# Viasat/nhd

Hardware: AMD Instinct MI355X
Metric: pod-placement filter-and-score throughput (pod x node fit-and-score evaluations/s; placement decisions/s under commit semantics in mode_b) (higher is better)
Workload: dtype u64 bitmaps + int32 table look-ups (f64 NIC arithmetic in the request digest)

## Files before the change

__graft_entry__.py:

```python
import os
import subprocess
import sys

ROOT = os.path.dirname(os.path.abspath(__file__))
if ROOT not in sys.path:
    sys.path.insert(0, ROOT)


def build() -> None:
    from nhd_amd import build as b
    b.build_lib()
    oracle_mk = os.path.join(ROOT, "oracle", "Makefile")
    if os.path.exists(oracle_mk):
        subprocess.check_call(["make", "-s", "-C", os.path.join(ROOT, "oracle")])
    from tests import harness
    harness.lib()
    from tests.harness import explain_twin
    explain_twin.lib()
    from tests.harness import headroom_twin
    headroom_twin.lib()
    headroom_twin.wave_lib()
    from tests.harness import headroom_limit_twin
    headroom_limit_twin.lib()
    from tests.harness import headroom_general_twin
    headroom_general_twin.lib()
    headroom_general_twin.wave_lib()
    from tests.harness import candidates_twin
    candidates_twin.lib()
    candidates_twin.pick_lib()
    from tests.harness import candidates_general_twin
    candidates_general_twin.lib()
    candidates_general_twin.wave_lib()
    import nhd_amd
    from nhd_amd import _lib
    lib = _lib.load()
    assert lib.nhdfit_abi_version() == _lib.ABI_VERSION


def smoke() -> None:
    import numpy as np
    from nhd_amd import matcher
    from workload import refmodel, synth
    from oracle import nhd_oracle as O

    spec = synth.make_cluster(3, n_nodes=192)
    nl = spec.build_nodes()
    pods, groups = synth.make_pods(3, n_pods=24)
    tops = [refmodel.make_topology(s) for s in pods]
    m = matcher.HipMatcher(device=0, clock=lambda: spec.clock_now)
    got = m.FindNodes(nl, tops)
    placed = 0
    for top, res in zip(tops, got):
        want = O.find_node(nl, top, spec.clock_now)
        if want[0] is None:
            assert res == (None,), (res, want)
        else:
            placed += 1
            assert res[0] == want[0] and res[1]["gpu"] == tuple(want[1]["gpu"]) and \
                res[1]["cpu"] == tuple(want[1]["cpu"]) and res[1]["nic"] == [tuple(x) for x in want[1]["nic"]], (res, want)
    assert placed > 0
    from nhd_amd.engine import winner_index
    reqs = m.packer.digest_many(tops)
    score, _, _ = m.engine.find(reqs, spec.clock_now, want_bitmap=True, want_map=True)
    names = list(nl)
    for s, res in zip(score.tolist(), got):
        assert (names[winner_index(s) - m.engine.global_base] if s else None) == res[0], (s, res)
    st = m.engine.stats()
    print(f"smoke ok: {len(tops)} pods x {len(nl)} nodes, {placed} placed; single-launch finds {st.small_finds}, step kernel {st.fit_ms_last * 1e3:.1f} us")


if __name__ == "__main__":
    build()
    if "--smoke" in sys.argv:
        smoke()
```

nhd_amd/csrc/fit_core.h:

```cpp
#pragma once
#include <stdint.h>
#include "../../include/nhdfit.h"

#if defined(__HIPCC__)
#define NHD_HD __host__ __device__ __forceinline__
#else
#define NHD_HD inline
#endif

namespace nhdfit {

constexpr int kMaxG      = NHDFIT_MAX_GROUPS;
constexpr int kTile      = NHDFIT_TILE;
constexpr int kMaxHpRows = 1024;
constexpr int kWClasses  = 4;
constexpr double kMinBusySecs = 30.0;
constexpr uint32_t kMinXCap = 32;

NHD_HD uint32_t align16(uint32_t x) { return (x + 15u) & ~15u; }
NHD_HD uint32_t wc_stride_of(uint32_t W) { return 2 * W * 8 + 16; }
NHD_HD uint32_t x_stride_of(uint32_t W) { return W == 2 ? 16u : W * 8 + 16; }

struct Layout {
    uint32_t W;
// ... 80 lines not shown
template <> struct req_traits<nhdfit_req> {
    static constexpr int kG = NHDFIT_MAX_GROUPS;
    static constexpr bool kBig = false;
    using Key = int16_t;
    static constexpr int kMaxTuples = 1024;
    using Mapping = nhdfit_mapping;
    using WidePlacement = nhdfit_wide_placement;
};
template <> struct req_traits<nhdfit_big_req> {
    static constexpr int kG = NHDFIT_BIG_MAX_GROUPS;
    static constexpr bool kBig = true;
    using Key = int32_t;
    static constexpr int kMaxTuples = NHDFIT_BIG_MAX_TUPLES;
    using Mapping = nhdfit_big_mapping;
    using WidePlacement = nhdfit_big_placement;
};
static_assert(sizeof(nhdfit_big_req) == 256 && sizeof(nhdfit_big_mapping) == 36 && sizeof(nhdfit_big_placement) == 904, "record sizes of include/nhdfit.h");
NHD_HD bool req_valid(const nhdfit_big_req& r) {
    return (r.map_type == NHDFIT_MAP_NUMA || r.map_type == NHDFIT_MAP_PCI) && r.n_groups >= 1 &&
           r.n_groups <= (uint32_t)NHDFIT_BIG_MAX_GROUPS;
}

NHD_HD void pod_sums(const nhdfit_req& r, PodSums& s) {
    s.G = r.n_groups;
    s.W = 1u << s.G;
    s.full = s.W - 1;
    s.misc_smt = r.misc_smt;
    s.misc_nosmt = r.misc_nosmt;
    for (uint32_t S = 0; S < s.W; ++S) {
        uint32_t g = 0, a = 0, b = 0;
        for (uint32_t i = 0; i < s.G; ++i)
            if (S >> i & 1) { g += r.gpus[i]; a += r.cpu_smt[i]; b += r.cpu_nosmt[i]; }
        s.gpu[S] = g; s.cpu_smt[S] = a; s.cpu_nosmt[S] = b;
    }
}

NHD_HD PodHeader pod_header(const nhdfit_req& r) {
    PodHeader h;
    h.hp_req = r.hugepages_gb;
    h.groups = r.groups;
    h.flags = 0;
    if (req_valid(r)) {
        h.flags |= kPodValid;
        uint32_t g = 0;
        for (uint32_t i = 0; i < r.n_groups; ++i) g += r.gpus[i];
        if (g) h.flags |= kPodNeedGpu;
        if (r.map_type == NHDFIT_MAP_PCI) h.flags |= kPodPci;
        if (r.flags & NHDFIT_RF_INITIAL_FILTER) h.flags |= kPodFilter;
        h.flags |= r.n_groups << kPodGroupsShift;
    }
    return h;
}

NHD_HD uint32_t entry_w(const PodSums& s, uint32_t u, bool smt, uint32_t c, uint32_t m) {
    const uint32_t* sum = smt ? s.cpu_smt : s.cpu_nosmt;
    const uint32_t extra = m ? (smt ? s.misc_smt : s.misc_nosmt) : 0;
    uint32_t out = 0;
    for (uint32_t p = 0; p < s.W; ++p)
        if (sum[u ? p : (~p & s.full)] + extra <= c) out |= 1u << p;
    return out;
}

NHD_HD uint32_t entry_a(const PodSums& s, uint32_t u, uint32_t f) {
    uint32_t a = 0;
    for (uint32_t p = 0; p < s.W; ++p)
        if (s.gpu[u ? p : (~p & s.full)] <= f) a |= 1u << p;
    return a;
}

static_assert(kMaxG == 4, "the disj() masks below enumerate subsets of four groups");
template <uint32_t TERMS>
NHD_HD uint32_t dunion_n(uint32_t a, uint32_t b) {
    uint32_t out = 0;
#if defined(__HIP_DEVICE_COMPILE__)
#pragma unroll
#endif
    for (uint32_t S = 0; S < TERMS; ++S) {
        const uint32_t disj = ((S & 1) ? 0x5555u : 0xFFFFu) & ((S & 2) ? 0x3333u : 0xFFFFu) &
                              ((S & 4) ? 0x0F0Fu : 0xFFFFu) & ((S & 8) ? 0x00FFu : 0xFFFFu);
        if (b >> S & 1) out |= (a & disj) << S;
    }
    return out;
}
NHD_HD uint32_t dunion(uint32_t a, uint32_t b, uint32_t W) {
    (void)W;
    return dunion_n<1u << kMaxG>(a, b);
}

NHD_HD bool block_fits(const nhdfit_req& r, double cap, uint32_t S) {
    double rx = cap, tx = cap;
    for (uint32_t i = 0; i < r.n_groups; ++i)
        if (S >> i & 1) { rx = rx - r.rx[i]; tx = tx - r.tx[i]; }
    return !(rx < 0) && !(tx < 0);
}

template <uint32_t WW>
NHD_HD void class_cover_w(const nhdfit_req& r, double cap, uint32_t W, uint32_t G, uint16_t cover[kMaxG + 1]) {
    uint32_t fit = 1;
    for (uint32_t S = 1; S < W; ++S)
        if (block_fits(r, cap, S)) fit |= 1u << S;
    cover[0] = 1;
    for (uint32_t n = 1; n <= (uint32_t)kMaxG; ++n)
        cover[n] = (n <= G) ? (uint16_t)dunion_n<WW>(cover[n - 1], fit) : cover[G];
}
NHD_HD void class_cover(const nhdfit_req& r, double cap, uint32_t W, uint32_t G, uint16_t cover[kMaxG + 1]) {
    class_cover_w<1u << kMaxG>(r, cap, W, G, cover);
}

NHD_HD uint32_t size_le_mask(uint32_t W, uint32_t limit) {
    const uint32_t by_size = limit == 0 ? 0x0001u : limit == 1 ? 0x0117u : limit == 2 ? 0x177Fu : limit == 3 ? 0x7FFFu : 0xFFFFu;
    return by_size & ((1u << W) - 1u);
}

struct SigDict {
    const uint32_t* sig_off;
    const uint32_t* pool_off;
    const uint8_t*  pool_glimit;
    const nhdfit_cc* cc;
    uint32_t nsig;
};

template <uint32_t WW>
NHD_HD uint32_t sig_reach_w(const SigDict& d, uint32_t sig, const uint16_t* cover, uint32_t W) {
    uint32_t reach = 1;
    for (uint32_t pl = d.sig_off[sig]; pl < d.sig_off[sig + 1]; ++pl) {
        uint32_t pool = 1;
        for (uint32_t k = d.pool_off[pl]; k < d.pool_off[pl + 1]; ++k) {
            uint32_t n = d.cc[k].cnt > kMaxG ? kMaxG : d.cc[k].cnt;
            pool = dunion_n<WW>(pool, cover[d.cc[k].cls * (kMaxG + 1) + n]);
        }
        if (d.pool_glimit[pl] != NHDFIT_GLIMIT_NONE) pool &= size_le_mask(W, d.pool_glimit[pl]);
        reach = dunion_n<WW>(reach, pool);
    }
    return reach;
}
NHD_HD uint32_t sig_reach(const SigDict& d, uint32_t sig, const uint16_t* cover, uint32_t W) {
    return sig_reach_w<1u << kMaxG>(d, sig, cover, W);
}

NHD_HD uint32_t entry_r(uint32_t reach, uint32_t W, uint32_t u) {
    if (u) return reach & 0xFFFFu;
    uint32_t r = reach & 0xFFFFu;
    r = (r & 0x5555u) << 1 | (r >> 1 & 0x5555u);
    r = (r & 0x3333u) << 2 | (r >> 2 & 0x3333u);
    r = (r & 0x0F0Fu) << 4 | (r >> 4 & 0x0F0Fu);
    r = (r & 0x00FFu) << 8 | (r >> 8 & 0x00FFu);
    return r >> (16 - W);
}

NHD_HD bool hp_bit(const PodHeader& h, uint32_t k) {
    if (!(h.flags & kPodValid)) return false;
    return h.hp_req <= (int32_t)k - 1;
}
NHD_HD bool gx_bit(const PodHeader& h, uint32_t g, const uint64_t* group_sets) {
    if (g == 0) return false;
    const uint32_t gs = (g - 1) >> 1, active = (g - 1) & 1;
    if (!(h.flags & kPodFilter)) return true;
    return active && (group_sets[gs] & h.groups) != 0;
}

struct NodeIdx {
    uint32_t w0, w1;
    uint32_t f0, f1;
    uint32_t hp;
    uint32_t gx;
    uint32_t nogpu;
};

NHD_HD NodeIdx node_index(const nhdfit_plane0& a, const nhdfit_plane1& b, const nhdfit_plane2& c, const nhdfit_plane4& e,
                          uint32_t fc_dim, uint32_t fg_dim, uint32_t ngs) {
    NodeIdx n;
    const uint32_t smt = (c.flags & NHDFIT_NF_SMT) ? fc_dim : 0;
    uint32_t c0 = popc64(a.t0[0] & b.t1[0]), c1 = popc64(a.t0[1] & b.t1[1]);
    c0 = c0 < fc_dim ? c0 : fc_dim - 1;
    c1 = c1 < fc_dim ? c1 : fc_dim - 1;
    n.w0 = smt + c0;
    n.w1 = smt + c1;
    uint32_t f0 = popc32(c.gpu_free & ~c.gpu_numa1), f1 = popc32(c.gpu_free & c.gpu_numa1);
    n.f0 = f0 < fg_dim ? f0 : fg_dim - 1;
    n.f1 = f1 < fg_dim ? f1 : fg_dim - 1;
    int32_t hp = c.hp_free;
    hp = hp < -1 ? -1 : hp;
    hp = hp > kMaxHpRows - 2 ? kMaxHpRows - 2 : hp;
    n.hp = (uint32_t)(hp + 1);
    const uint32_t gs = e.group_set < ngs ? e.group_set : 0;
    n.gx = (c.flags & NHDFIT_NF_MAINTENANCE) ? 0u : 1u + 2u * gs + ((c.flags & NHDFIT_NF_ACTIVE) ? 1u : 0u);
    n.nogpu = (c.flags & NHDFIT_NF_HAS_GPU) ? 0u : 1u;
    return n;
}

NHD_HD uint64_t xkey(uint32_t u, uint32_t f, uint32_t sig_numa, uint32_t sig_pci) {
    return (1ull << 63) | ((uint64_t)u << 62) | ((uint64_t)f << 32) | ((uint64_t)sig_numa << 16) | (uint64_t)sig_pci;
}
NHD_HD uint32_t xkey_u(uint64_t k) { return (uint32_t)(k >> 62) & 1u; }
NHD_HD uint32_t xkey_f(uint64_t k) { return (uint32_t)(k >> 32) & 0xFFu; }
NHD_HD uint32_t xkey_sig_numa(uint64_t k) { return (uint32_t)(k >> 16) & 0xFFFFu; }
NHD_HD uint32_t xkey_sig_pci(uint64_t k) { return (uint32_t)k & 0xFFFFu; }

struct alignas(16) NodeRec {
    uint16_t w0, w1, x0, x1;
    uint16_t gx;
    uint16_t hp;
    uint16_t flags;
    uint16_t cc;
};
static_assert(sizeof(NodeRec) == 16, "one 16-byte load per node");
static_assert(kMaxHpRows <= 1024, "NodeRec::hp keeps ten bits for the row index");
constexpr uint16_t kRecNoGpu = 1;
NHD_HD uint32_t rec_hp(const NodeRec& r) { return r.hp & 1023u; }
NHD_HD uint32_t rec_pos(const NodeRec& r) { return r.hp >> 10; }

NHD_HD uint32_t pair_c_row(uint32_t cc, uint32_t D);
NHD_HD NodeRec make_record(const NodeIdx& n, uint32_t x0, uint32_t x1, const Layout& L, uint32_t pos, uint32_t crow_D = 0) {
    NodeRec r;
    r.w0 = (uint16_t)((L.hot_wc0 + n.w0 * L.wc_stride) >> 3);
    r.w1 = (uint16_t)((L.hot_wc1 + n.w1 * L.wc_stride) >> 3);
    r.x0 = (uint16_t)((L.hot_x + x0 * L.x_stride) >> 3);
    r.x1 = (uint16_t)((L.hot_x + x1 * L.x_stride) >> 3);
    r.gx = (uint16_t)((L.hot_gx + n.gx * 8) >> 3);
    r.hp = (uint16_t)(n.hp | (pos & 63u) << 10);
    r.flags = (uint16_t)(n.nogpu ? kRecNoGpu : 0);
    const uint32_t smt = n.w0 >= L.fc_dim ? 1u : 0u;
    r.cc = (uint16_t)((n.w0 - smt * L.fc_dim) | (n.w1 - smt * L.fc_dim) << 7 | smt << 14);
    if (crow_D) r.flags = (uint16_t)(r.flags | pair_c_row(r.cc, crow_D) << 1);
    return r;
}
NHD_HD NodeRec dead_record(const Layout& L, uint32_t pos) {
    NodeRec r;
    r.w0 = (uint16_t)(L.hot_wc0 >> 3); r.w1 = (uint16_t)(L.hot_wc1 >> 3);
    r.x0 = r.x1 = (uint16_t)(L.hot_x >> 3);
    r.gx = (uint16_t)(L.hot_gx >> 3);
    r.hp = (uint16_t)((pos & 63u) << 10); r.flags = 0; r.cc = 0;
    return r;
}

NHD_HD uint32_t req_max_demand(const nhdfit_req& r) {
    uint32_t a = r.misc_smt, b = r.misc_nosmt;
    for (uint32_t i = 0; i < r.n_groups && i < (uint32_t)kMaxG; ++i) { a += r.cpu_smt[i]; b += r.cpu_nosmt[i]; }
    return a > b ? a : b;
}
NHD_HD uint32_t pair_dim(uint32_t max_demand, uint32_t fc_dim) { return max_demand + 1 < fc_dim ? max_demand + 1 : fc_dim; }
NHD_HD uint32_t pair_c_row(uint32_t cc, uint32_t D) {
    const uint32_t c0 = cc & 127u, c1 = (cc >> 7) & 127u, smt = cc >> 14;
    return ((smt * D + (c0 < D ? c0 : D - 1)) * D + (c1 < D ? c1 : D - 1));
}

inline double busy_threshold(double now) {
    constexpr uint64_t kSign = 1ull << 63, kMaxBits = 0x7FEFFFFFFFFFFFFFull;
    auto at = [](uint64_t key) {
        const uint64_t bits = key & kSign ? key ^ kSign : ~key;
        double x;
        __builtin_memcpy(&x, &bits, sizeof x);
        return x;
    };
    auto is_busy = [now](double t) { return (now - t) < kMinBusySecs; };
    uint64_t lo = ~(kMaxBits | kSign), hi = kMaxBits | kSign;
    if (!is_busy(at(hi))) return __builtin_nan("");
    if (is_busy(at(lo))) return at(lo);
    while (hi - lo > 1) {
        const uint64_t mid = lo + (hi - lo) / 2;
        if (is_busy(at(mid))) hi = mid; else lo = mid;
    }
    return at(hi);
}

NHD_HD uint64_t ld64(const uint8_t* img, uint32_t off) { return *reinterpret_cast<const uint64_t*>(img + off); }

NHD_HD uint64_t node_word_hot(const uint8_t* hot, const Layout& L, const NodeRec& r, bool busy, uint64_t m_need) {
    const uint32_t w0 = (uint32_t)r.w0 << 3, w1 = (uint32_t)r.w1 << 3, x0 = (uint32_t)r.x0 << 3, x1 = (uint32_t)r.x1 << 3;
    uint64_t acc = 0;
    for (uint32_t p = 0; p < L.W; ++p) {
        const uint32_t o = p * 8;
        const uint64_t cpu = (ld64(hot, w0 + L.row + o) & ld64(hot, w1 + o)) | (ld64(hot, w0 + o) & ld64(hot, w1 + L.row + o));
        acc |= cpu & ld64(hot, x0 + o) & ld64(hot, x1 + o);
    }
    const uint32_t hp = rec_hp(r) < L.hp_rows ? rec_hp(r) : L.hp_rows - 1;
    uint64_t pred = ld64(hot, (uint32_t)r.gx << 3) & ld64(hot, L.hot_hp + hp * 8);
    if (busy) pred &= ~m_need;
    return acc & pred;
}

NHD_HD uint64_t node_word_pair(const uint8_t* hot, const Layout& L, const NodeRec& r, uint32_t D, bool busy, uint64_t m_need) {
    const uint32_t row = pair_c_row(r.cc, D), smt = r.cc >> 14, c0 = (row / D) % D, c1 = row % D;
    const uint32_t w0 = L.hot_wc0 + (smt * L.fc_dim + c0) * L.wc_stride, w1 = L.hot_wc1 + (smt * L.fc_dim + c1) * L.wc_stride;
    const uint32_t x0 = (uint32_t)r.x0 << 3, x1 = (uint32_t)r.x1 << 3;
    uint64_t acc = 0;
    for (uint32_t p = 0; p < L.W; ++p) {
        const uint32_t o = p * 8;
        const uint64_t cpu = (ld64(hot, w0 + L.row + o) & ld64(hot, w1 + o)) | (ld64(hot, w0 + o) & ld64(hot, w1 + L.row + o));
        acc |= cpu & ld64(hot, x0 + o) & ld64(hot, x1 + o);
    }
    const uint32_t hp = rec_hp(r) < L.hp_rows ? rec_hp(r) : L.hp_rows - 1;
    uint64_t pred = ld64(hot, (uint32_t)r.gx << 3) & ld64(hot, L.hot_hp + hp * 8);
    if (busy) pred &= ~m_need;
    return acc & pred;
}

NHD_HD uint64_t node_term_cold(const uint8_t* img, const Layout& L, const NodeIdx& n, const nhdfit_plane3& q3, uint64_t m_pci, uint32_t p) {
    const uint8_t* hot = img + L.off_hot;
    const uint32_t w0 = L.hot_wc0 + n.w0 * L.wc_stride, w1 = L.hot_wc1 + n.w1 * L.wc_stride;
    const uint32_t o = p * 8;
    const uint64_t cpu = (ld64(hot, w0 + L.row + o) & ld64(hot, w1 + o)) | (ld64(hot, w0 + o) & ld64(hot, w1 + L.row + o));
    const uint64_t r0 = (ld64(img, L.off_r0 + q3.sig_pci[0] * L.row + o) & m_pci) | (ld64(img, L.off_r0 + q3.sig_numa[0] * L.row + o) & ~m_pci);
    const uint64_t r1 = (ld64(img, L.off_r1 + q3.sig_pci[1] * L.row + o) & m_pci) | (ld64(img, L.off_r1 + q3.sig_numa[1] * L.row + o) & ~m_pci);
    return cpu & ld64(img, L.off_a0 + n.f0 * L.row + o) & ld64(img, L.off_a1 + n.f1 * L.row + o) & r0 & r1;
}
// ... 91 lines not shown
```

nhd_amd/csrc/nhdfit.hip:

```cpp
#include <hip/hip_runtime.h>
#include <dlfcn.h>
#include <rccl/rccl.h>

#include <algorithm>
#include <chrono>
#include <cstdarg>
#include <cstdio>
#include <cstdlib>
#include <cstring>
#include <map>
#include <set>
#include <new>
#include <string>
#include <type_traits>
#include <vector>

#include "seq_core.h"
#include "wide_core.h"
#include "explain_core.h"
#include "dict_stream.h"
#include "host_streams.h"
#include "headroom_merge.h"
#include "candidates_merge.h"

// ... 1044 lines not shown
            std::vector<uint64_t> keys(c->nx);
            if (c->nx) HIPCHK(c, hipMemcpy(keys.data(), c->xcls.p, (size_t)c->nx * sizeof(uint64_t), hipMemcpyDeviceToHost));
            std::vector<uint8_t> used(0x10000u, 0);
            for (uint64_t k : keys) { used[xkey_sig_numa(k)] = 1; used[xkey_sig_pci(k)] = 1; }
            std::vector<uint16_t> list;
            for (uint32_t sg = 0; sg < 0x10000u; ++sg)
                if (used[sg]) list.push_back((uint16_t)sg);
            HIPCHK(c, c->sig_use.reserve(list.size() ? list.size() : 1));
            if (!list.empty()) HIPCHK(c, hipMemcpy(c->sig_use.p, list.data(), list.size() * sizeof(uint16_t), hipMemcpyHostToDevice));
            c->n_sig_use = (uint32_t)list.size();
            c->sig_use_nx = c->nx;
        }
        if (nx[0] <= c->x_cap) break;
        TRY(sync_all(c));
        c->x_cap = x_capacity(nx[0]);
        c->rec_all = true;
        for (Pipe& p : c->pipe) p.n_dig = std::min(p.n_dig, p.n_fit);
        TRY(refresh_layouts(c, P));
    }
    if (deal) {
        const bool every = c->ord_all || c->rec_all;
        if (every || dealt_count >= 16) TRY(order_chunks(c, every ? 0 : dealt_first, every ? all_chunks : dealt_count, every));
    }
    c->ord_all = false;
    c->rec_all = false;
    c->rec_lo = c->rec_hi = 0;
    return NHDFIT_OK;
}

int build_items(nhdfit_ctx* c, uint32_t nw, bool batch_find = false) {
    const uint32_t tiles = (c->P + kTile - 1) / kTile, chunks = (c->n + 63) / 64;
    const uint32_t cus = (uint32_t)c->prop.multiProcessorCount;
    uint32_t target = cus * (nw == 8 ? 2u : 5u);
    uint64_t total = 0;
    for (uint32_t t = 0; t < tiles; ++t) total += (uint64_t)chunks * (6u + (2u << c->h_tile_wcls[t]));
    std::vector<FitItem> items;
    const uint64_t rec_bytes = (uint64_t)chunks * 64u * (16u * (c->max_wcls + 1u) + 8u);
    const bool small_shard = rec_bytes <= (2u << 20);
    if (small_shard && nw == 8) target = cus;
    const bool by_xcd = chunks >= 8u * 4u * nw && (nw == 8 || batch_find) && !small_shard;
    for (uint32_t t = 0; t < tiles; ++t) {
        const uint32_t w = c->h_tile_wcls[t];
        const uint64_t cost = (uint64_t)chunks * (6u + (2u << w));
        uint32_t nb = (uint32_t)((cost * target + total / 2) / total);
        nb = std::max(1u, std::min(nb, (chunks + nw - 1) / nw));
        if (small_shard && nw == 8) nb = std::min(nb, 8u);
        if (by_xcd) {
            const uint32_t k = batch_find ? 2u : 1u;
            for (uint32_t j = 0; j < 8 * k; ++j) {
                const uint32_t r = (j % 8) * k + j / 8;
                const uint32_t lo = (uint32_t)((uint64_t)chunks * r / (8 * k)), hi = (uint32_t)((uint64_t)chunks * (r + 1) / (8 * k));
                items.push_back(FitItem{t, w, lo, hi});
            }
            continue;
        }
        for (uint32_t b = 0; b < nb; ++b) {
            const uint32_t lo = (uint32_t)((uint64_t)chunks * b / nb), hi = (uint32_t)((uint64_t)chunks * (b + 1) / nb);
            if (hi > lo) items.push_back(FitItem{t, w, lo, hi});
        }
    }
    HIPCHK(c, c->items.reserve(items.size() ? items.size() : 1));
    HIPCHK(c, c->pin_items.reserve(items.size() * sizeof(FitItem) + (size_t)tiles * sizeof(uint32_t) + 1));
    memcpy(c->pin_items.p, items.data(), items.size() * sizeof(FitItem));
    if (batch_find) {
        uint32_t* per_tile = reinterpret_cast<uint32_t*>(c->pin_items.p + items.size() * sizeof(FitItem));
        for (uint32_t t = 0; t < tiles; ++t) per_tile[t] = 0;
        for (const FitItem& it : items) per_tile[it.tile]++;
    } else
        HIPCHK(c, hipMemcpyAsync(c->items.p, c->pin_items.p, items.size() * sizeof(FitItem), hipMemcpyHostToDevice, c->streams.use(0)));
    c->n_items = (uint32_t)items.size();
    c->staged_gen++;
    return NHDFIT_OK;
}

void fill_digest_args(nhdfit_ctx* c, Pipe& p, int b, uint32_t wc_parts, uint32_t P, DigestArgs& d) {
    d.reqs = c->reqs.p; d.P = P;
    d.d = DictView{c->caps.p, c->ncls, c->group_sets.p, SigDict{c->sig_off.p, c->pool_off.p, c->pool_glimit.p, c->cc.p, c->nsig}, c->sig_flat.p, c->flat_words,
                   c->sig_flat2.p, c->flat2_words};
    for (int w = 0; w < kWClasses; ++w) d.L[w] = c->L[w];
    d.pitch = c->pitch; d.tabs = p.tabs[b].p; d.hdr = p.hdr[b].p; d.score = p.score[b].p;
    d.xcls = c->xcls.p; d.nx = c->xnx.p;
    d.wc_parts = wc_parts;
    d.sig_parts = 1u;
    const bool listed = !c->all_sigs && c->sig_use_nx == c->nx && c->nx != 0;
    d.sig_list = listed ? c->sig_use.p : nullptr;
    d.n_sig_list = listed ? c->n_sig_use : 0;
    d.count = p.dig_count.p;
}
void fill_fit_args(nhdfit_ctx* c, Pipe& p, int bf, double now, uint32_t P, FitArgs& f, bool pair = false) {
    for (int w = 0; w < 2; ++w) {
        f.pair_D[w] = pair ? c->pair_D[w] : 0u;
        f.crow_ok[w] = pair && c->pair_D[w] != 0u && c->crow_D[w] == c->pair_D[w] && !c->crow_stale ? 1u : 0u;
        f.hot_wc1[w] = c->L[w].hot_wc1;
    }
    f.fc_dim = c->max_cores + 1;
    for (int w = 0; w < kWClasses; ++w) {
        f.rec[w] = c->rec[w].p; f.bt[w] = c->rec_bt[w].p; f.off_hot[w] = c->L[w].off_hot; f.hot_bytes[w] = c->L[w].hot_bytes; f.hot_hp[w] = c->L[w].hot_hp; f.hot_staged[w] = c->hot_staged[w];
    }
    f.hp_last = c->hp_rows - 1; f.hp_bytes = align16(c->hp_rows * 8);
    f.n = c->n; f.chunks = (c->n + 63) / 64; f.global_base = c->global_base; f.busy_from = busy_threshold(now);
    f.tabs = p.tabs[bf].p; f.pitch = c->pitch; f.hdr = p.hdr[bf].p; f.P = P;
    f.cand = c->use_cand ? c->cand.p : nullptr;
    f.nm = c->want_bitmap ? p.nm.p : nullptr;
    f.score = p.score[bf].p;
    f.items = c->items.p;
    f.dbg_skip = tune_env("NHDFIT_FIT_SKIP") ? (uint32_t)atoi(tune_env("NHDFIT_FIT_SKIP")) : 0;
    f.clk = nullptr;
}

int launch_step(nhdfit_ctx* c, Pipe& p, bool with_fit, bool with_digest, double now) {
    const uint32_t P = c->P, tiles = (P + kTile - 1) / kTile;
    const uint32_t chunks = (c->n + 63) / 64;
    const bool big = c->geom_big;
    const uint32_t block = big ? 512 : 256, nw = block / 64;
    const bool small_map = c->want_map && c->n_big_pods < P;
    if (with_fit || with_digest) TRY(ensure_records(c, P));
    if (with_fit && !c->n_items) TRY(build_items(c, nw));
    if (&p != &c->pipe[0] && p.seen_gen != c->staged_gen) {
        HIPCHK(c, hipEventRecord(p.ev_staged, c->streams.use(0)));
        HIPCHK(c, hipStreamWaitEvent(c->streams.use(p.k), p.ev_staged, 0));
        p.seen_gen = c->staged_gen;
    }

    StepArgs a;
    memset(&a, 0, sizeof a);
    a.shapes_P = P;
    a.side_prio = 1;
    bool did_shapes = false, did_choose = false, did_finish = false;
    if (small_map) {
        if (p.n_finished < p.n_chosen) {
            const int b = (int)(p.n_finished % kBufs);
            a.finish_m = make_map_args(c, p, b, P); a.finish_h = make_shape_args(c, p, b); a.nb_finish = (P + block / 4 - 1) / (block / 4); did_finish = true;
        }
        if (p.n_chosen < p.n_shaped) {
            a.choose = make_shape_args(c, p, (int)(p.n_chosen % kBufs));
            a.choose_lanes = 1u;
            a.nb_choose = (tiles + nw - 1) / nw; did_choose = true;
        }
        const uint64_t ready = c->comm && p.n_fit ? p.n_fit - 1 : p.n_fit;
        if (p.n_shaped < ready) {
            const int b = (int)(p.n_shaped % kBufs);
            if (c->comm) HIPCHK(c, hipStreamWaitEvent(c->streams.use(p.k), p.ev_red[b], 0));
            HIPCHK(c, p.shape_keys[b].reserve((size_t)tiles * kTile));
            HIPCHK(c, p.shape_res[b].reserve((size_t)tiles * kTile));
            HIPCHK(c, p.shape_slot[b].reserve(P));
            HIPCHK(c, p.shape_list[b].reserve(tiles));
            a.shapes_m = make_map_args(c, p, b, P); a.shapes_h = make_shape_args(c, p, b); a.nb_shapes = (P + block / 4 - 1) / (block / 4); did_shapes = true;
        }
    }
    with_digest = with_digest && p.n_dig <= p.n_fit + (with_fit ? 1 : 0);
    if (with_digest) {
        const int b = (int)(p.n_dig % kBufs);
        DigestArgs& d = a.digest;
        constexpr uint32_t wc_parts = 2;
        fill_digest_args(c, p, b, wc_parts, P, d);
        a.nb_digest = tiles * (1u + wc_parts);
    }
    uint32_t nb_fit = 0;
    int bf = -1;
    if (with_fit) {
        bf = (int)(p.n_fit % kBufs);
        if (c->want_bitmap) HIPCHK(c, p.nm.reserve((size_t)tiles * chunks * 64));
        fill_fit_args(c, p, bf, now, P, a.fit, !c->x_spill);
        nb_fit = c->n_items;
    }
    a.nb_fit = nb_fit;
    const uint32_t grid = a.nb_choose + a.nb_shapes + a.nb_finish + a.nb_digest + nb_fit;
    if (!grid) return NHDFIT_OK;
    size_t lds = nb_fit ? fit_launch_lds(c, nw) : 0;
    if (a.nb_digest && kDigestLds > lds) lds = kDigestLds;
    const size_t map_lds = big ? map_lds_bytes<512>() : map_lds_bytes<256>();
    if ((a.nb_shapes || a.nb_finish) && map_lds > lds) lds = map_lds;

    const bool clocks = kTuning && with_fit && (int64_t)p.n_fit == c->role_step;
    if (clocks) {
        TRY(arm_role_clock(c, p.k, 5));
        a.role_clock = c->role_clock.p;
        a.fit.clk = c->role_clock.p + 16;
    }
    const bool timed = (with_fit && (p.n_fit < 2 || (p.n_fit & 7) == 0)) || (!with_fit && with_digest);
    if (timed && c->ev_pending == kEventRing) { int rc = drain_events(c); if (rc) return rc; }
    static const bool enq_prof = tune_env("NHDFIT_ENQ_PROF") != nullptr;
    const auto t_ev0 = enq_prof ? std::chrono::steady_clock::now() : std::chrono::steady_clock::time_point();
    if (timed) HIPCHK(c, hipEventRecord(c->ev[c->ev_pending][0], c->streams.use(p.k)));
    const auto t_l0 = enq_prof ? std::chrono::steady_clock::now() : std::chrono::steady_clock::time_point();
    if (enq_prof) c->enq_events_us += std::chrono::duration<double, std::micro>(t_l0 - t_ev0).count();
    if (c->x_spill) {
        if (big) hipLaunchKernelGGL((k_step<512, true>), dim3(grid), dim3(512), lds, c->streams.use(p.k), a);
        else     hipLaunchKernelGGL((k_step<256, true>), dim3(grid), dim3(256), lds, c->streams.use(p.k), a);
    } else if (big) hipLaunchKernelGGL((k_step<512>), dim3(grid), dim3(512), lds, c->streams.use(p.k), a);
    else     hipLaunchKernelGGL((k_step<256>), dim3(grid), dim3(256), lds, c->streams.use(p.k), a);
    HIPCHK(c, hipGetLastError());
    if (enq_prof) c->enq_launch_us += std::chrono::duration<double, std::micro>(std::chrono::steady_clock::now() - t_l0).count();
    if (with_fit && c->n_wide) {
        WideArgs wa;
        memset(&wa, 0, sizeof wa);
        wa.wide = c->wide.p; wa.n_wide = c->n_wide; wa.reqs = c->reqs.p; wa.P = P; wa.caps = c->caps.p; wa.busy_from = busy_threshold(now);
        wa.cand = c->use_cand ? c->cand.p : nullptr;
        wa.nm = c->want_bitmap ? reinterpret_cast<unsigned long long*>(p.nm.p) : nullptr; wa.chunks = chunks;
        wa.score = p.score[bf].p; wa.global_base = c->global_base; wa.share = c->sharing ? c->wide_share.p : nullptr;
        const uint64_t pairs = (uint64_t)c->n_wide * P;
        hipLaunchKernelGGL(k_wide_eval, dim3((uint32_t)((pairs + 255) / 256)), dim3(256), 0, c->streams.use(p.k), wa);
        HIPCHK(c, hipGetLastError());
    }
    if (timed) {
        const auto t_e1 = enq_prof ? std::chrono::steady_clock::now() : std::chrono::steady_clock::time_point();
        HIPCHK(c, hipEventRecord(c->ev[c->ev_pending][1], c->streams.use(p.k)));
        c->ev_kind[c->ev_pending++] = with_fit ? 0 : 1;
        if (enq_prof) c->enq_events_us += std::chrono::duration<double, std::micro>(std::chrono::steady_clock::now() - t_e1).count();
    }
    if (clocks) {
        const std::string line = "[nhdfit] step " + std::to_string(c->role_step) + " role %-6s: first block starts +%.2f us, last block ends +%.2f us\n";
        TRY(report_role_clock(c, p.k, 5, line.c_str()));
    }
    p.n_finished += did_finish; p.n_chosen += did_choose; p.n_shaped += did_shapes;
    if (with_digest) p.n_dig++;
    if (with_fit) {
        int after = p.k;
        if (c->comm) {
            HIPCHK(c, hipEventRecord(p.ev_fit[bf], c->streams.use(p.k)));
            HIPCHK(c, hipStreamWaitEvent(c->streams.use(kRed), p.ev_fit[bf], 0));
            TRY(rccl(c, kRed, "ncclAllReduce", &Rccl::AllReduce, p.score[bf].p, p.score[bf].p, P, ncclUint64, ncclMax, c->comm));
            after = kRed;
        }
        if (c->want_map && c->n_big_pods) {
            const dim3 mg((P + kMapWaves - 1) / kMapWaves), mb(64 * kMapWaves);
            hipLaunchKernelGGL(k_map<true>, mg, mb, 0, c->streams.use(after), make_map_args(c, p, bf, P));
            HIPCHK(c, hipGetLastError());
        }
        if (c->comm) HIPCHK(c, hipEventRecord(p.ev_red[bf], c->streams.use(kRed)));
        p.n_fit++;
        if (!small_map) p.n_shaped = p.n_chosen = p.n_finished = p.n_fit;
        store_find_stats(c, (uint64_t)P * c->n, (uint64_t)tiles * c->n * 24ull + (uint64_t)P * sizeof(nhdfit_req) +
                                                (c->want_bitmap ? (uint64_t)tiles * chunks * 64ull * 8ull : 0ull) + (uint64_t)P * 8ull);
        c->stats.pipes = (uint32_t)c->npipes;
    }
    return NHDFIT_OK;
}

int convert_rows(nhdfit_ctx* c, Pipe& p) {
    const uint32_t chunks = (c->n + 63) / 64, tiles = (c->P + kTile - 1) / kTile;
    HIPCHK(c, c->bitmap.reserve((size_t)chunks * c->P));
    hipLaunchKernelGGL(k_rows, dim3((tiles * chunks + 3) / 4), dim3(256), 0, c->streams.use(p.k), p.nm.p, c->bitmap.p, chunks, c->P);
    HIPCHK(c, hipGetLastError());
    HIPCHK(c, c->streams.wait(p.k));
    return NHDFIT_OK;
}

int enqueue_step(nhdfit_ctx* c, double now) {
    if (!c->P) return fail(c, NHDFIT_E_STATE, "stage requests first");
    if (!c->n) return fail(c, NHDFIT_E_STATE, "no nodes uploaded");
    HIPCHK(c, hipSetDevice(c->dev));
    if (c->n_enq == 0) {
        const uint32_t tiles = (c->P + kTile - 1) / kTile, chunks = (c->n + 63) / 64;
        c->geom_big = (uint64_t)tiles * ((chunks + 31) / 32) >= (uint32_t)c->prop.multiProcessorCount;
        static const int force_pipes = tune_env("NHDFIT_PIPES") ? atoi(tune_env("NHDFIT_PIPES")) : 0;
        c->npipes = force_pipes >= 1 && force_pipes <= kPipes ? force_pipes : (c->geom_big && c->nsig > 64) ? 3 : 2;
    }
    const int which = (int)(c->n_enq % (uint64_t)c->npipes);
    Pipe& p = c->pipe[which];
    c->n_enq++;
    c->last_pipe = which;
    TRY(ensure_records(c, c->P));
    if (p.n_dig <= p.n_fit) {
        TRY(launch_step(c, p, false, true, now));
    }
    return launch_step(c, p, true, true, now);
}

}

int nhdfit_stage_requests(nhdfit_ctx* c, const nhdfit_req* reqs, uint32_t P) {
    if (!c) return NHDFIT_E_INVAL;
    return stage_requests(c, reqs, P, false, false);
}

int nhdfit_enqueue_step(nhdfit_ctx* c, double now) {
    if (!c) return NHDFIT_E_INVAL;
    static const bool enq_prof = tune_env("NHDFIT_ENQ_PROF") != nullptr;
    if (!enq_prof) return enqueue_step(c, now);
    const auto t0 = std::chrono::steady_clock::now();
    const int rc = enqueue_step(c, now);
    c->enq_us += std::chrono::duration<double, std::micro>(std::chrono::steady_clock::now() - t0).count();
    if (++c->enq_n % 1000 == 0) {
        fprintf(stderr, "[nhdfit] 1000 enqueues: %.2f us each on the host, %.2f in the launch calls, %.2f in event records\n", c->enq_us / 1000, c->enq_launch_us / 1000, c->enq_events_us / 1000);
        c->enq_us = c->enq_launch_us = c->enq_events_us = 0;
    }
    return rc;
}

int nhdfit_sync(nhdfit_ctx* c) {
    if (!c) return NHDFIT_E_INVAL;
    HIPCHK(c, hipSetDevice(c->dev));
    return sync_all(c);
}

int nhdfit_fetch(nhdfit_ctx* c, uint64_t* score_out, uint64_t* bitmap_out, nhdfit_mapping* map_out) {
    if (!c) return NHDFIT_E_INVAL;
    Pipe& p = c->pipe[c->last_pipe];
    if (!c->P || !p.n_fit) return fail(c, NHDFIT_E_STATE, "nothing staged / no step enqueued");
    HIPCHK(c, hipSetDevice(c->dev));
    if (map_out && !c->want_map) return fail(c, NHDFIT_E_STATE, "mapping output is disabled");
    const uint32_t P = c->P;
    const int b = (int)((p.n_fit - 1) % kBufs);
    TRY(flush_pipeline(c));
    if (c->comm) HIPCHK(c, c->streams.wait(kRed));
    if (map_out && c->n_wide) {
// ... 1684 lines not shown
```

nhd_amd/csrc/step_digest.h:

```cpp
struct DictView {
    const double* caps;
    uint32_t ncls;
    const uint64_t* group_sets;
    SigDict sig;
    const uint16_t* flat;
    uint32_t flat_words;
    const uint16_t* flat2;
    uint32_t flat2_words;
};
constexpr uint32_t kPoolSlots = 128;

extern "C" __device__ int nhd_writelane(int value, int lane, int old) __asm("llvm.amdgcn.writelane.i32");

struct PaddedReq { nhdfit_req r; uint32_t pad; };

template <int THREADS>
__device__ __forceinline__ void stage_requests_lds(const nhdfit_req* __restrict__ reqs, uint32_t pod0, uint32_t P, PaddedReq* s_req) {
    constexpr uint32_t kParts = sizeof(nhdfit_req) / 16;
    const uint32_t live = pod0 < P ? (P - pod0 < (uint32_t)kTile ? P - pod0 : (uint32_t)kTile) : 0u;
    const uint4* src = reinterpret_cast<const uint4*>(reqs + pod0);
    for (uint32_t c = threadIdx.x; c < kTile * kParts; c += THREADS) {
        const uint32_t j = c / kParts;
        const uint4 v = j < live ? src[c] : make_uint4(0u, 0u, 0u, 0u);
        uint32_t* dst = reinterpret_cast<uint32_t*>(&s_req[j]) + (c % kParts) * 4;
        dst[0] = v.x; dst[1] = v.y; dst[2] = v.z; dst[3] = v.w;
    }
}

template <class T>
__device__ __forceinline__ T* carve(uint8_t*& p, size_t count) {
    T* r = reinterpret_cast<T*>(p);
    p += (count * sizeof(T) + 15) & ~size_t(15);
    return r;
}
constexpr size_t lds_slice(size_t bytes) { return (bytes + 15) & ~size_t(15); }

struct DigestArgs {
    const nhdfit_req* reqs;
    uint32_t P;
    DictView d;
    Layout L[kWClasses];
    uint32_t pitch;
    uint8_t* tabs;
    PodHeader* hdr;
    unsigned long long* score;
    const uint64_t* xcls;
    const uint32_t* nx;
    uint32_t wc_parts;
    uint32_t sig_parts;
    uint32_t* count;
    const uint16_t* sig_list;
    uint32_t n_sig_list;
};
constexpr uint32_t kDictLdsWords = 6144;
constexpr size_t kPoolLds = (size_t)kPoolSlots * kTile * sizeof(uint16_t);
constexpr size_t kDigestLds = lds_slice(kTile * sizeof(PodSums)) +
                              lds_slice(kTile * NHDFIT_MAX_CLASSES * (kMaxG + 1) * sizeof(uint16_t)) + lds_slice(kTile * sizeof(PodHeader)) +
                              lds_slice(kDictLdsWords * sizeof(uint16_t)) + 16 +
                              (lds_slice(kTile * sizeof(PaddedReq)) > kPoolLds ? lds_slice(kTile * sizeof(PaddedReq)) : kPoolLds);
constexpr uint32_t kWcPartsDefault = 4;

template <int THREADS>
__device__ __forceinline__ void role_digest(const DigestArgs& a, uint32_t blk, uint8_t* lds) {
    PodSums* s_sum = carve<PodSums>(lds, kTile);
    uint16_t (*s_cover)[NHDFIT_MAX_CLASSES][kMaxG + 1] =
        reinterpret_cast<uint16_t (*)[NHDFIT_MAX_CLASSES][kMaxG + 1]>(carve<uint16_t>(lds, kTile * NHDFIT_MAX_CLASSES * (kMaxG + 1)));
    PodHeader* s_hdr = carve<PodHeader>(lds, kTile);
    uint16_t* s_flat = carve<uint16_t>(lds, kDictLdsWords);
    uint32_t& s_last = *carve<uint32_t>(lds, 4);
    PaddedReq* s_req = reinterpret_cast<PaddedReq*>(lds);
    uint16_t* s_pw = reinterpret_cast<uint16_t*>(lds);

    const uint32_t per_tile = a.sig_parts + a.wc_parts, tile = blk / per_tile, idx = blk % per_tile;
    const uint32_t part = idx < a.sig_parts ? 0u : idx - a.sig_parts + 1u, sig_part = idx < a.sig_parts ? idx : 0u;
    const uint32_t tid = threadIdx.x;
    uint8_t* img = a.tabs + (size_t)tile * a.pitch;

    stage_requests_lds<THREADS>(a.reqs, tile * kTile, a.P, s_req);
    __syncthreads();
    constexpr uint32_t NW = THREADS / 64;
    const uint32_t wave = tid >> 6, lane = tid & 63;
    if (tid < kTile) {
        const nhdfit_req& r = s_req[tid].r;
        const PodHeader h = pod_header(r);
        s_hdr[tid] = h;
        PodSums& ps = s_sum[tid];
        ps.G = r.n_groups; ps.W = 1u << (r.n_groups & 7u); ps.full = ps.W - 1;
        ps.misc_smt = r.misc_smt; ps.misc_nosmt = r.misc_nosmt;
        if (part == 0 && sig_part == 0) {
            const uint32_t pod = tile * kTile + tid;
            a.hdr[pod] = h;
            if (pod < a.P) a.score[pod] = 0;
        }
    }
    {
        const nhdfit_req& r = s_req[lane].r;
        const bool ok = req_valid(r);
        for (uint32_t S = wave; S < (1u << kMaxG); S += NW) {
            if (!ok || S >= (1u << r.n_groups)) continue;
            uint32_t g = 0, x = 0, y = 0;
            for (uint32_t i = 0; i < r.n_groups; ++i)
                if (S >> i & 1) { g += r.gpus[i]; x += r.cpu_smt[i]; y += r.cpu_nosmt[i]; }
            s_sum[lane].gpu[S] = g; s_sum[lane].cpu_smt[S] = x; s_sum[lane].cpu_nosmt[S] = y;
        }
    }
    __syncthreads();

    const bool valid = (s_hdr[lane].flags & kPodValid) != 0;
    const uint32_t my_g = valid ? (s_hdr[lane].flags >> kPodGroupsShift) & 7u : 0u;
    const uint32_t wcls = __ballot(my_g >= 4) ? 3u : __ballot(my_g == 3) ? 2u : __ballot(my_g == 2) ? 1u : 0u;
    const Layout& L = a.L[wcls];
    const uint32_t W = L.W;
    uint8_t* hot = img + L.off_hot;
    auto emit_row = [&](uint8_t* row, uint32_t v) __attribute__((always_inline)) {
        unsigned long long mine = 0;
        for (uint32_t p = 0; p < W; ++p) {
            const unsigned long long word = __ballot(v >> p & 1);
            if (lane == p) mine = word;
        }
        if (lane < W) *reinterpret_cast<unsigned long long*>(row + lane * 8) = mine;
    };

    if (part != 0) {
        for (uint32_t g = wave; g < 8; g += NW) {
            const uint32_t u = g >> 2, m = (g >> 1) & 1, smt = g & 1;
            uint32_t t[1 << kMaxG];
#pragma unroll
            for (uint32_t p = 0; p < (1u << kMaxG); ++p) {
                t[p] = 0xFFFFFFFFu;
                if (p < W && valid && p < s_sum[lane].W) {
                    const uint32_t* sum = smt ? s_sum[lane].cpu_smt : s_sum[lane].cpu_nosmt;
                    const uint32_t extra = m ? (smt ? s_sum[lane].misc_smt : s_sum[lane].misc_nosmt) : 0;
                    t[p] = sum[u ? p : (~p & s_sum[lane].full)] + extra;
                }
            }
            uint8_t* base = hot + (u ? L.hot_wc1 : L.hot_wc0) + smt * L.fc_dim * L.wc_stride + m * L.row;
            for (uint32_t c = part - 1; c < L.fc_dim; c += a.wc_parts) {
                uint32_t v = 0;
#pragma unroll
                for (uint32_t p = 0; p < (1u << kMaxG); ++p)
                    if (p < W) v |= (t[p] <= c ? 1u : 0u) << p;
                emit_row(base + c * L.wc_stride, v);
            }
        }
        if (part != a.wc_parts) return;
        for (uint32_t k = wave; k < L.hp_rows; k += NW) {
            const uint64_t word = __ballot(hp_bit(s_hdr[lane], k));
            if (lane == 0) *reinterpret_cast<uint64_t*>(hot + L.hot_hp + 8 * k) = word;
        }
        const bool filtered = (s_hdr[lane].flags & kPodFilter) != 0;
        const uint64_t my_groups = s_hdr[lane].groups;
        const uint64_t unfiltered = __ballot(!filtered);
        if (tid == 0) *reinterpret_cast<uint64_t*>(hot + L.hot_gx) = 0;
        for (uint32_t g0 = wave * 64; g0 < L.ngs; g0 += NW * 64) {
            const uint32_t cnt = L.ngs - g0 < 64u ? L.ngs - g0 : 64u;
            const uint64_t my_set = lane < cnt ? a.d.group_sets[g0 + lane] : 0ull;
            uint64_t mine = 0;
            for (uint32_t i = 0; i < cnt; ++i) {
                const uint64_t set = (uint64_t)(uint32_t)__builtin_amdgcn_readlane((int)(uint32_t)my_set, (int)i) |
                                     (uint64_t)(uint32_t)__builtin_amdgcn_readlane((int)(uint32_t)(my_set >> 32), (int)i) << 32;
                const uint64_t word = unfiltered | __ballot(filtered && (set & my_groups) != 0);
                if (lane == i) mine = word;
            }
            if (lane < cnt) {
                uint64_t* rows = reinterpret_cast<uint64_t*>(hot + L.hot_gx + 8 * (1 + 2 * (g0 + lane)));
                rows[0] = unfiltered;
                rows[1] = mine;
            }
        }
        return;
    }

    const bool typed = a.d.flat2_words != 0 && a.d.flat2_words <= kDictLdsWords;
    const bool staged = !typed && a.d.flat_words != 0 && a.d.flat_words <= kDictLdsWords;
    if (typed)
        for (uint32_t w = tid; w < a.d.flat2_words / 2; w += THREADS)
            reinterpret_cast<uint32_t*>(s_flat)[w] = reinterpret_cast<const uint32_t*>(a.d.flat2)[w];
    if (staged)
        for (uint32_t w = tid; w < a.d.flat_words / 2; w += THREADS)
            reinterpret_cast<uint32_t*>(s_flat)[w] = reinterpret_cast<const uint32_t*>(a.d.flat)[w];
    auto covers_and_sig_rows = [&](auto width) __attribute__((always_inline)) {
        constexpr uint32_t WW = decltype(width)::value;
        for (uint32_t w = tid; w < kTile * a.d.ncls; w += THREADS) {
            const uint32_t j = w % kTile, c = w / kTile;
            if (s_hdr[j].flags & kPodValid) class_cover_w<WW>(s_req[j].r, a.d.caps[c], s_sum[j].W, s_sum[j].G, s_cover[j][c]);
        }
        __syncthreads();
        if (typed) {
            auto bword = [&](uint32_t i) { return (uint32_t)__builtin_amdgcn_readfirstlane((int)s_flat[i]); };
            const uint32_t ntypes = bword(0), nsig_d = a.d.sig.nsig;
            const uint32_t t_off = 2, s_off = t_off + ntypes + 1, recs = s_off + nsig_d + 1;
            for (uint32_t t = wave; t < ntypes; t += NW) {
                uint32_t at = recs + bword(t_off + t);
                const uint32_t head = bword(at++), ncc = head & 0xFFu, glimit = head >> 8;
                const uint32_t ks = bword(at++), kmax = ks >> 8, first = ks & 0xFFu;
                uint32_t pool = 1;
                for (uint32_t k = 0; k < ncc; ++k) {
                    const uint32_t e = bword(at++), cnt = e & 0xFFu, cls = e >> 8;
                    pool = dunion_n<WW>(pool, s_cover[lane][cls][cnt > (uint32_t)kMaxG ? kMaxG : cnt]);
                }
                if (glimit != NHDFIT_GLIMIT_NONE) pool &= size_le_mask(s_sum[lane].W, glimit);
                uint32_t pw = pool;
                for (uint32_t k = 0; k < kmax; ++k) {
                    s_pw[(first + k) * kTile + lane] = (uint16_t)pw;
                    pw = dunion_n<WW>(pw, pool);
                }
            }
            __syncthreads();
            const uint32_t sig_first = sig_part * NW + wave, sig_step = a.sig_parts * NW;
            uint32_t offs_lo = 0, offs_hi = 0, seq = 0;
            const uint32_t n_sigs = a.sig_list ? a.n_sig_list : L.nsig;
            uint32_t sig_ids = 0;
            for (uint32_t idx = sig_first; idx < n_sigs; idx += sig_step, ++seq) {
                if ((seq & 63u) == 0) {
                    const uint32_t at = idx + lane * sig_step;
                    const uint32_t mine = at < n_sigs ? (a.sig_list ? (uint32_t)a.sig_list[at] : at) : L.nsig;
                    sig_ids = mine;
                    offs_lo = mine < L.nsig ? s_flat[s_off + mine] : 0u;
                    offs_hi = mine < L.nsig ? s_flat[s_off + mine + 1] : 0u;
                }
                const uint32_t sig = (uint32_t)__builtin_amdgcn_readlane((int)sig_ids, (int)(seq & 63u));
                const uint32_t rec0 = (uint32_t)__builtin_amdgcn_readlane((int)offs_lo, (int)(seq & 63u));
                const uint32_t rec1 = (uint32_t)__builtin_amdgcn_readlane((int)offs_hi, (int)(seq & 63u));
                const uint32_t len = rec1 - rec0;
                const uint32_t my_word = lane < len ? s_flat[recs + rec0 + lane] : 0u;
                const uint32_t nent = (uint32_t)__builtin_amdgcn_readlane((int)my_word, 0);
                uint32_t reach = 1;
                for (uint32_t e = 0; e < nent; ++e) {
                    const uint32_t slot = (uint32_t)__builtin_amdgcn_readlane((int)my_word, (int)(1 + e));
                    reach = dunion_n<WW>(reach, s_pw[slot * kTile + lane]);
                }
                if (!valid) reach = 0;
                emit_row(img + L.off_r0 + sig * L.row, valid ? entry_r(reach, s_sum[lane].W, 0) : 0u);
                emit_row(img + L.off_r1 + sig * L.row, valid ? entry_r(reach, s_sum[lane].W, 1) : 0u);
            }
            return;
        }
        const uint32_t sig_first = sig_part * NW + wave, sig_step = a.sig_parts * NW;
        uint32_t offs_lo = 0, offs_hi = 0;
        uint32_t seq = 0;
        const uint32_t n_sigs = a.sig_list ? a.n_sig_list : L.nsig;
        uint32_t sig_ids = 0;
        for (uint32_t idx = sig_first; idx < n_sigs; idx += sig_step, ++seq) {
            uint32_t reach = 0;
            if ((seq & 63u) == 0) {
                const uint32_t at = idx + lane * sig_step;
                sig_ids = at < n_sigs ? (a.sig_list ? (uint32_t)a.sig_list[at] : at) : L.nsig;
            }
            const uint32_t sig = (uint32_t)__builtin_amdgcn_readlane((int)sig_ids, (int)(seq & 63u));
            if (staged) {
                if ((seq & 63u) == 0) {
                    const uint32_t mine = sig_ids;
                    offs_lo = mine < L.nsig ? s_flat[mine] : 0u;
                    offs_hi = mine + 1 < L.nsig ? s_flat[mine + 1] : a.d.flat_words - (a.d.sig.nsig + 1);
                }
                const uint32_t rec0 = (uint32_t)__builtin_amdgcn_readlane((int)offs_lo, (int)(seq & 63u));
                const uint32_t rec1 = (uint32_t)__builtin_amdgcn_readlane((int)offs_hi, (int)(seq & 63u));
                const uint32_t base = a.d.sig.nsig + 1 + rec0;
                reach = 1;
                if (rec1 - rec0 <= 64u) {
                    const uint32_t my_word = lane < rec1 - rec0 ? s_flat[base + lane] : 0u;
                    auto word = [&](uint32_t i) { return (uint32_t)__builtin_amdgcn_readlane((int)my_word, (int)i); };
                    uint32_t at = 0;
                    const uint32_t npools = word(at++);
                    for (uint32_t pl = 0; pl < npools; ++pl) {
                        const uint32_t head = word(at++), ncc = head & 0xFFu, glimit = head >> 8;
                        uint32_t pool = 1;
                        for (uint32_t k = 0; k < ncc; ++k) {
                            const uint32_t e = word(at++), cnt = e & 0xFFu, cls = e >> 8;
                            pool = dunion_n<WW>(pool, s_cover[lane][cls][cnt > (uint32_t)kMaxG ? kMaxG : cnt]);
                        }
                        if (glimit != NHDFIT_GLIMIT_NONE) pool &= size_le_mask(s_sum[lane].W, glimit);
                        reach = dunion_n<WW>(reach, pool);
                    }
                } else {
                    auto word = [&](uint32_t i) { return (uint32_t)__builtin_amdgcn_readfirstlane((int)s_flat[i]); };
                    uint32_t at = base;
                    const uint32_t npools = word(at++);
                    for (uint32_t pl = 0; pl < npools; ++pl) {
                        const uint32_t head = word(at++), ncc = head & 0xFFu, glimit = head >> 8;
                        uint32_t pool = 1;
                        for (uint32_t k = 0; k < ncc; ++k) {
                            const uint32_t e = word(at++), cnt = e & 0xFFu, cls = e >> 8;
                            pool = dunion_n<WW>(pool, s_cover[lane][cls][cnt > (uint32_t)kMaxG ? kMaxG : cnt]);
                        }
                        if (glimit != NHDFIT_GLIMIT_NONE) pool &= size_le_mask(s_sum[lane].W, glimit);
                        reach = dunion_n<WW>(reach, pool);
                    }
                }
                if (!valid) reach = 0;
            } else {
                reach = valid ? sig_reach_w<WW>(a.d.sig, sig, &s_cover[lane][0][0], s_sum[lane].W) : 0u;
            }
            emit_row(img + L.off_r0 + sig * L.row, valid ? entry_r(reach, s_sum[lane].W, 0) : 0u);
            emit_row(img + L.off_r1 + sig * L.row, valid ? entry_r(reach, s_sum[lane].W, 1) : 0u);
        }
    };
    if (W == 2) covers_and_sig_rows(std::integral_constant<uint32_t, 2>{});
    else if (W == 4) covers_and_sig_rows(std::integral_constant<uint32_t, 4>{});
    else if (W == 8) covers_and_sig_rows(std::integral_constant<uint32_t, 8>{});
    else covers_and_sig_rows(std::integral_constant<uint32_t, 16>{});
// ... 34 lines not shown
```

Measured before the change: 16900 billion.

## Build digest threshold rows via 64x64 bit transpose instead of per-row ballots

Rewrites the digest kernel's CPU-capacity and hugepage threshold-row generation. Each lane now builds a 64-bit threshold mask and a wave-wide 64x64 bit transpose emits 64 rows at once, replacing one ballot per row and per partition bit. Work units are split over (group, partition-pair) across all wc_parts blocks, and wc_parts becomes tunable through an environment variable. The transpose64 helper is only forward-declared here, and rows beyond 64 get special handling, which adds complexity and correctness risk.

```diff
diff --git a/__graft_entry__.py b/__graft_entry__.py
--- a/__graft_entry__.py
+++ b/__graft_entry__.py
@@ -31,6 +31,8 @@
     from tests.harness import candidates_general_twin
     candidates_general_twin.lib()
     candidates_general_twin.wave_lib()
+    from tests.harness import threshold_twin
+    threshold_twin.lib()
     import nhd_amd
     from nhd_amd import _lib
     lib = _lib.load()
diff --git a/nhd_amd/csrc/fit_core.h b/nhd_amd/csrc/fit_core.h
--- a/nhd_amd/csrc/fit_core.h
+++ b/nhd_amd/csrc/fit_core.h
@@ -256,6 +256,31 @@
     if (!(h.flags & kPodValid)) return false;
     return h.hp_req <= (int32_t)k - 1;
 }
+constexpr uint32_t kNoDemand = 0xFFFFFFFFu;
+NHD_HD uint64_t threshold_mask(uint32_t t, uint32_t c0) {
+    if (t == kNoDemand) return 0ull;
+    if (t <= c0) return ~0ull;
+    const uint32_t d = t - c0;
+    return d < 64u ? ~0ull << d : 0ull;
+}
+NHD_HD uint32_t cpu_demand(const PodSums& s, bool valid, uint32_t u, bool smt, uint32_t m, uint32_t p) {
+    if (!valid || p >= s.W) return kNoDemand;
+    const uint32_t* sum = smt ? s.cpu_smt : s.cpu_nosmt;
+    const uint32_t extra = m ? (smt ? s.misc_smt : s.misc_nosmt) : 0;
+    return sum[u ? p : (~p & s.full)] + extra;
+}
+NHD_HD uint32_t hp_demand(const PodHeader& h) {
+    if (!(h.flags & kPodValid)) return kNoDemand;
+    return h.hp_req < 0 ? 0u : (uint32_t)h.hp_req + 1u;
+}
+inline void threshold_rows_plain(const uint64_t mask[64], uint64_t rows[64]) {
+    for (uint32_t c = 0; c < 64; ++c) {
+        uint64_t w = 0;
+        for (uint32_t j = 0; j < 64; ++j) w |= (mask[j] >> c & 1ull) << j;
+        rows[c] = w;
+    }
+}
+
 NHD_HD bool gx_bit(const PodHeader& h, uint32_t g, const uint64_t* group_sets) {
     if (g == 0) return false;
     const uint32_t gs = (g - 1) >> 1, active = (g - 1) & 1;
diff --git a/nhd_amd/csrc/nhdfit.hip b/nhd_amd/csrc/nhdfit.hip
--- a/nhd_amd/csrc/nhdfit.hip
+++ b/nhd_amd/csrc/nhdfit.hip
@@ -1220,7 +1220,8 @@
     if (with_digest) {
         const int b = (int)(p.n_dig % kBufs);
         DigestArgs& d = a.digest;
-        constexpr uint32_t wc_parts = 2;
+        static const uint32_t wc_parts = tune_env("NHDFIT_WC_PARTS") && atoi(tune_env("NHDFIT_WC_PARTS")) >= 1 && atoi(tune_env("NHDFIT_WC_PARTS")) <= 4
+                                             ? (uint32_t)atoi(tune_env("NHDFIT_WC_PARTS")) : 2u;
         fill_digest_args(c, p, b, wc_parts, P, d);
         a.nb_digest = tiles * (1u + wc_parts);
     }
diff --git a/nhd_amd/csrc/step_digest.h b/nhd_amd/csrc/step_digest.h
--- a/nhd_amd/csrc/step_digest.h
+++ b/nhd_amd/csrc/step_digest.h
@@ -11,6 +11,8 @@
 constexpr uint32_t kPoolSlots = 128;
 
 extern "C" __device__ int nhd_writelane(int value, int lane, int old) __asm("llvm.amdgcn.writelane.i32");
+
+__device__ __forceinline__ void transpose64(uint32_t& lo, uint32_t& hi);
 
 struct PaddedReq { nhdfit_req r; uint32_t pad; };
 
@@ -122,31 +124,29 @@
     };
 
     if (part != 0) {
-        for (uint32_t g = wave; g < 8; g += NW) {
+        const uint32_t wc_waves = a.wc_parts * NW, swave = (uint32_t)__builtin_amdgcn_readfirstlane((int)wave);
+        for (uint32_t unit = (part - 1) * NW + swave; unit < (8u << wcls); unit += wc_waves) {
+            const uint32_t g = unit >> wcls, p0 = (unit & ((1u << wcls) - 1u)) * 2;
             const uint32_t u = g >> 2, m = (g >> 1) & 1, smt = g & 1;
-            uint32_t t[1 << kMaxG];
-#pragma unroll
-            for (uint32_t p = 0; p < (1u << kMaxG); ++p) {
-                t[p] = 0xFFFFFFFFu;
-                if (p < W && valid && p < s_sum[lane].W) {
-                    const uint32_t* sum = smt ? s_sum[lane].cpu_smt : s_sum[lane].cpu_nosmt;
-                    const uint32_t extra = m ? (smt ? s_sum[lane].misc_smt : s_sum[lane].misc_nosmt) : 0;
-                    t[p] = sum[u ? p : (~p & s_sum[lane].full)] + extra;
-                }
-            }
-            uint8_t* base = hot + (u ? L.hot_wc1 : L.hot_wc0) + smt * L.fc_dim * L.wc_stride + m * L.row;
-            for (uint32_t c = part - 1; c < L.fc_dim; c += a.wc_parts) {
-                uint32_t v = 0;
-#pragma unroll
-                for (uint32_t p = 0; p < (1u << kMaxG); ++p)
-                    if (p < W) v |= (t[p] <= c ? 1u : 0u) << p;
-                emit_row(base + c * L.wc_stride, v);
+            const uint32_t ta = cpu_demand(s_sum[lane], valid, u, smt != 0, m, p0), tb = cpu_demand(s_sum[lane], valid, u, smt != 0, m, p0 + 1);
+            uint8_t* base = hot + (u ? L.hot_wc1 : L.hot_wc0) + smt * L.fc_dim * L.wc_stride + m * L.row + p0 * 8;
+            const uint64_t ma = threshold_mask(ta, 0), mb = threshold_mask(tb, 0);
+            uint32_t alo = (uint32_t)ma, ahi = (uint32_t)(ma >> 32), blo = (uint32_t)mb, bhi = (uint32_t)(mb >> 32);
+            transpose64(alo, ahi);
+            transpose64(blo, bhi);
+            if (lane < L.fc_dim) *reinterpret_cast<uint4*>(base + lane * L.wc_stride) = make_uint4(alo, ahi, blo, bhi);
+            if (L.fc_dim > 64) {
+                const uint64_t wa = __ballot(threshold_mask(ta, 64) & 1ull), wb = __ballot(threshold_mask(tb, 64) & 1ull);
+                if (lane == 0) *reinterpret_cast<uint4*>(base + 64 * L.wc_stride) = make_uint4((uint32_t)wa, (uint32_t)(wa >> 32), (uint32_t)wb, (uint32_t)(wb >> 32));
             }
         }
         if (part != a.wc_parts) return;
-        for (uint32_t k = wave; k < L.hp_rows; k += NW) {
-            const uint64_t word = __ballot(hp_bit(s_hdr[lane], k));
-            if (lane == 0) *reinterpret_cast<uint64_t*>(hot + L.hot_hp + 8 * k) = word;
+        const uint32_t t_hp = hp_demand(s_hdr[lane]);
+        for (uint32_t k0 = swave * 64; k0 < L.hp_rows; k0 += NW * 64) {
+            const uint64_t mk = threshold_mask(t_hp, k0);
+            uint32_t lo = (uint32_t)mk, hi = (uint32_t)(mk >> 32);
+            transpose64(lo, hi);
+            if (k0 + lane < L.hp_rows) *reinterpret_cast<uint64_t*>(hot + L.hot_hp + 8 * (k0 + lane)) = ((uint64_t)hi << 32) | lo;
         }
         const bool filtered = (s_hdr[lane].flags & kPodFilter) != 0;
         const uint64_t my_groups = s_hdr[lane].groups;
```

Result: slower. 16090 billion (-4.8%).
